# pyannote/pyannote-video

Hardware: AMD Instinct MI355X
Metric: frames/sec end-to-end detect->embed->cluster, 1080p@25fps (higher is better)
Workload: dtype f32 (detector scores, embedder) / f64 (tracker, clustering) / u8 frames; an f16 screening pass with a proven error bound decides which windows the detector's exact f32 chain is evaluated for -- results identical to dense f32 scoring (`dense_scoring`)

## Files before the change

include/pvface.h:

```cpp
#ifndef PVFACE_H
#define PVFACE_H
#include <stdint.h>
#include <stddef.h>

#ifdef __cplusplus
extern "C" {
#endif

typedef uint64_t pvf_handle;
typedef struct { int32_t left, top, right, bottom; } pvf_rect_i32;

const char* pvf_last_error(void);
int32_t pvf_version(void);
int32_t pvf_device_count(int32_t* n);
int32_t pvf_ctx_create(int32_t device, pvf_handle* ctx);
int32_t pvf_ctx_create_prio(int32_t device, int32_t priority_class, pvf_handle* ctx);
int32_t pvf_ctx_destroy(pvf_handle ctx);
int32_t pvf_sync(pvf_handle ctx);

int32_t pvf_load_detector(pvf_handle ctx, const char* path);
int32_t pvf_load_shape_predictor(pvf_handle ctx, const char* path);
int32_t pvf_load_embedder(pvf_handle ctx, const char* path);
int32_t pvf_model_tensor(const char* path, int32_t kind, const char* name, void* out, int64_t cap_bytes, int64_t* nbytes);
int32_t pvf_set_tracker_tables(pvf_handle ctx, const double* mask64, const double* mask_scale, const double* tw64,
// ... 22 lines not shown
#define PVF_PRIM_RECT 0
#define PVF_PRIM_LINE 1
#define PVF_PRIM_TEXT 2
#define PVF_RENDER_MAX_PRIMS 4096
#define PVF_RENDER_MAX_RUN 64
#define PVF_RENDER_MAX_TEXT (1 << 20)
#define PVF_RENDER_MAX_SCALE 64
#define PVF_RENDER_MAX_BATCH 1024
typedef struct { int32_t type, a, b, c, d; uint32_t colour; int32_t scale, reserved; } pvf_prim;
int32_t pvf_render_batch(pvf_handle ctx, const pvf_handle* frames, int32_t n, int32_t out_w, int32_t out_h, int32_t flags,
                         const int32_t* start, const pvf_prim* prims, const uint8_t* text, int64_t text_bytes,
                         uint8_t* out, int32_t out_on_device);
int32_t pvf_egress_create(pvf_handle ctx, int32_t out_w, int32_t out_h, int32_t depth, int32_t flags, pvf_handle* ring);
int32_t pvf_egress_destroy(pvf_handle ctx, pvf_handle ring);
int32_t pvf_egress_submit(pvf_handle ctx, pvf_handle ring, pvf_handle frame, const pvf_prim* prims, int32_t n_prims,
                          const uint8_t* text, int64_t text_bytes, int32_t* slot);
int32_t pvf_egress_wait(pvf_handle ctx, pvf_handle ring, int32_t slot, const uint8_t** host_planes);
int32_t pvf_egress_release(pvf_handle ctx, pvf_handle ring, int32_t slot);
int32_t pvf_debug_render_rgb(pvf_handle ctx, pvf_handle frame, int32_t out_w, int32_t out_h, const pvf_prim* prims, int32_t n_prims,
                             const uint8_t* text, int64_t text_bytes, uint8_t* rgb);

int32_t pvf_detect(pvf_handle ctx, pvf_handle frame, int32_t upsample, double adjust_threshold,
                   pvf_rect_i32* out, float* scores, int32_t cap, int32_t* n);
int32_t pvf_detect_batch(pvf_handle ctx, const pvf_handle* frames, int32_t n_frames, int32_t upsample,
                         double adjust_threshold, pvf_rect_i32* out, float* scores, int32_t* counts,
                         int32_t cap_per_frame);
int32_t pvf_detect_many(pvf_handle ctx, const pvf_handle* frames, int32_t n_frames, int32_t batch, int32_t upsample,
                        double adjust_threshold, pvf_rect_i32* out, float* scores, int32_t* counts, int32_t cap);

int32_t pvf_detector_screening(pvf_handle ctx, int32_t on, int32_t list_cap);
int32_t pvf_detector_screening_stats(pvf_handle ctx, int64_t* batches, int64_t* listed, int64_t* retries, double* bounds, double* pipe_err);

int32_t pvf_embedder_split(pvf_handle ctx, int32_t on);
int32_t pvf_embedder_split_stats(pvf_handle ctx, int64_t* faces, int64_t* reruns, double* pipe_err);

int32_t pvf_tracker_create(pvf_handle ctx, pvf_handle* trk);
int32_t pvf_tracker_create_many(pvf_handle ctx, int32_t n, pvf_handle* trks);
int32_t pvf_tracker_destroy_many(pvf_handle ctx, const pvf_handle* trks, int32_t n);
int32_t pvf_tracker_clone_many(pvf_handle ctx, const pvf_handle* src, int32_t n, pvf_handle* dst);
int32_t pvf_tracker_destroy(pvf_handle ctx, pvf_handle trk);
int32_t pvf_tracker_start(pvf_handle ctx, pvf_handle trk, pvf_handle frame, const double box[4]);
int32_t pvf_tracker_update(pvf_handle ctx, pvf_handle trk, pvf_handle frame, double* psr);
int32_t pvf_tracker_position(pvf_handle ctx, pvf_handle trk, double box[4]);
int32_t pvf_tracker_start_many(pvf_handle ctx, const pvf_handle* trks, const pvf_handle* frames,
                               const double* boxes , int32_t n);
int32_t pvf_tracker_update_many(pvf_handle ctx, const pvf_handle* trks, const pvf_handle* frames, int32_t n,
                                double* psr , double* boxes_out );
int32_t pvf_tracker_update_many_deferred(pvf_handle ctx, const pvf_handle* trks, const pvf_handle* frames, int32_t n,
                                         double* psr, double* boxes_out);
int32_t pvf_tracker_commit_many(pvf_handle ctx, const pvf_handle* trks, const pvf_handle* frames, int32_t n);

int32_t pvf_overlap_matrix(const double* a, int32_t na, const double* b, int32_t nb, double ratio, double* out);
int32_t pvf_associate(const double* trackers, int32_t n_trackers, const double* detections, int32_t n_detections,
                      double min_overlap_ratio, int32_t* det_of_tracker);
int32_t pvf_munkres(const double* cost, int32_t n, int32_t* row_to_col);

int32_t pvf_landmarks(pvf_handle ctx, const pvf_handle* frames, const pvf_rect_i32* boxes, int32_t n,
                      int32_t* pts );
int32_t pvf_embed(pvf_handle ctx, const pvf_handle* frames, const int32_t* pts , int32_t n,
                  float* out );
int32_t pvf_landmarks_embed(pvf_handle ctx, const pvf_handle* frames, const pvf_rect_i32* boxes, int32_t n,
                            int32_t* pts , float* out );
int32_t pvf_embed_chips(pvf_handle ctx, const uint8_t* chips, int32_t n, float* out );
int32_t pvf_face_chips(pvf_handle ctx, const pvf_handle* frames, const int32_t* pts, int32_t n, uint8_t* chips );

#define PVF_JITTER_ROW 17
// ... 113 lines not shown
```

pyannote-video_amd/csrc/api.hip:

```cpp
#include "pvf_internal.h"
#include <algorithm>
#include <cmath>
#include <cstdlib>
#include <string>
#include <thread>

#define API_BEGIN try {
#define API_END                                                        \
    return 0;                                                          \
    }                                                                  \
    catch (const std::exception& e) { pvf_set_error(e.what()); return -1; } \
    catch (...) { pvf_set_error("unknown error"); return -2; }

#define ENTER(c, h)                                                \
    Ctx* c = pvf_ctx(h);                                           \
    std::lock_guard<std::recursive_mutex> _api_lock(c->api_mu);    \
    HIP_CHECK(hipSetDevice(c->device))
#define ENTER_DET(c, h)                                            \
    Ctx* c = pvf_ctx(h);                                           \
    std::lock_guard<std::recursive_mutex> _det_lock(c->det_mu);    \
    HIP_CHECK(hipSetDevice(c->device))
#define ENTER_BOTH(c, h)                                           \
    Ctx* c = pvf_ctx(h);                                           \
    std::lock_guard<std::recursive_mutex> _det_lock(c->det_mu);    \
// ... 19 lines not shown
            with_candidate_room(c, run);
            return;
        }
    }
}

extern "C" int32_t pvf_detector_screening(pvf_handle h, int32_t on, int32_t list_cap)
{
    API_BEGIN
    ENTER_DET(c, h);
    PVF_REQUIRE(list_cap >= 0 && list_cap <= (1 << 26), "pvf_detector_screening: list_cap must be 0 (keep) .. 2^26");
    c->det_screen = on != 0;
    if (list_cap > 0) c->screen_list_cap = list_cap;
    API_END
}

extern "C" int32_t pvf_detector_screening_stats(pvf_handle h, int64_t* batches, int64_t* listed, int64_t* retries, double* bounds, double* pipe_err)
{
    API_BEGIN
    ENTER_DET(c, h);
    if (batches) *batches = c->screen_batches;
    if (listed) *listed = c->screen_listed;
    if (retries) *retries = c->screen_retries;
    if (bounds) for (int f = 0; f < c->det.n_filters; ++f) bounds[f] = c->det.screen_bound[f];
    if (pipe_err) *pipe_err = c->screen_pipe_err;
    API_END
}

extern "C" int32_t pvf_embedder_split(pvf_handle h, int32_t on)
{
    API_BEGIN
    ENTER(c, h);
    c->emb_split = on != 0;
    API_END
}

extern "C" int32_t pvf_embedder_split_stats(pvf_handle h, int64_t* faces, int64_t* reruns, double* pipe_err)
{
    API_BEGIN
    ENTER(c, h);
    if (faces) *faces = c->emb_split_faces;
    if (reruns) *reruns = c->emb_reruns;
    if (pipe_err) *pipe_err = c->emb_pipe_err;
    API_END
}

extern "C" int32_t pvf_detect_batch(pvf_handle h, const pvf_handle* frames, int32_t n_frames, int32_t upsample, double adjust,
                                    pvf_rect_i32* out, float* scores, int32_t* counts, int32_t cap)
{
    API_BEGIN
    ENTER_DET(c, h);
    PVF_REQUIRE(n_frames > 0 && frames && out && counts && cap > 0, "pvf_detect_batch: bad arguments");
    PVF_REQUIRE(upsample >= 0 && upsample <= 2, "pvf_detect_batch: upsample must be 0..2");
    std::vector<Frame> fr(n_frames);
    for (int i = 0; i < n_frames; ++i) fr[i] = c->frame(frames[i]);
    std::vector<std::vector<RawDet>> raw;
    with_candidate_room(c, [&]() { det_run_batch(c, fr, upsample, adjust, raw); });
    std::vector<RawDet> kept;
    for (int i = 0; i < n_frames; ++i) {
        det_nms(c->det, raw[i], kept);
        const int n = std::min<int>((int)kept.size(), cap);
        counts[i] = n;
        for (int k = 0; k < n; ++k) {
            out[(size_t)i * cap + k] = pvf_rect_i32{kept[k].l, kept[k].t, kept[k].rr, kept[k].b};
            if (scores) scores[(size_t)i * cap + k] = kept[k].score;
        }
// ... 1135 lines not shown
```

pyannote-video_amd/csrc/ctx.hip:

```cpp
#include "pvf_internal.h"
#include "detect_ml.h"
#include <cmath>
#include <fstream>
#include <mutex>
#include <dlfcn.h>

static thread_local std::string g_err;
void pvf_set_error(const char* msg) { g_err = msg ? msg : ""; }
extern "C" const char* pvf_last_error(void) { return g_err.c_str(); }

static std::mutex g_ctx_mu;
static std::unordered_map<uint64_t, std::unique_ptr<Ctx>> g_ctxs;
static uint64_t g_next_ctx = 0x1000;

Ctx* pvf_ctx(pvf_handle h)
{
    std::lock_guard<std::mutex> lk(g_ctx_mu);
    auto it = g_ctxs.find(h);
    if (it == g_ctxs.end()) throw PvfError("unknown context handle");
    return it->second.get();
}

std::map<std::string, Tensor> pvf_read_container(const char* path)
{
// ... 236 lines not shown
{
    API_BEGIN
    int k = 0;
    hipError_t e = hipGetDeviceCount(&k);
    if (e != hipSuccess) k = 0;
    *n = k;
    API_END
}

extern "C" int32_t pvf_ctx_create_prio(int32_t device, int32_t priority_class, pvf_handle* out)
{
    API_BEGIN
    int k = 0;
    if (hipGetDeviceCount(&k) != hipSuccess || k <= 0) throw PvfError("no HIP device visible: libpvface has no CPU fallback");
    PVF_REQUIRE(device >= 0 && device < k, "device index out of range");
    HIP_CHECK(hipSetDevice(device));
    hipDeviceProp_t prop;
    HIP_CHECK(hipGetDeviceProperties(&prop, device));
    if (strncmp(prop.gcnArchName, "gfx950", 6) != 0)
        throw PvfError(std::string("libpvface is built for gfx950 (MI355X) only; device is ") + prop.gcnArchName);
    std::unique_ptr<Ctx> c(new Ctx());
    c->device = device;
    c->n_cu = prop.multiProcessorCount;
    {
        int lo = 0, hi = 0;
        HIP_CHECK(hipDeviceGetStreamPriorityRange(&lo, &hi));
        int prio = priority_class < 0 ? lo : hi;
        if (const char* e = getenv("PVF_MAIN_STREAM_PRIO")) prio = (strcmp(e, "low") == 0) ? lo : hi;
        HIP_CHECK(hipStreamCreateWithPriority(&c->stream, hipStreamNonBlocking, priority_class == 2 ? lo : prio));
        HIP_CHECK(hipStreamCreateWithPriority(&c->det_stream, hipStreamNonBlocking, priority_class == 2 ? hi : lo));
    }
    if (const char* e = getenv("PVF_DETECTOR_SCREENING")) c->det_screen = atoi(e) != 0;
    if (const char* e = getenv("PVF_EMBEDDER_SPLIT")) c->emb_split = atoi(e) != 0;
    std::lock_guard<std::mutex> lk(g_ctx_mu);
    uint64_t id = g_next_ctx++;
    g_ctxs[id] = std::move(c);
    *out = id;
    API_END
}

extern "C" int32_t pvf_ctx_create(int32_t device, pvf_handle* out) { return pvf_ctx_create_prio(device, 0, out); }

extern "C" int32_t pvf_ctx_destroy(pvf_handle h)
{
    API_BEGIN
    Ctx* c = pvf_ctx(h);
    HIP_CHECK(hipSetDevice(c->device));
    (void)hipStreamSynchronize(c->stream);
    (void)hipStreamSynchronize(c->det_stream);
    for (auto& kv : c->frames) if (kv.second.owned) (void)hipFree((void*)kv.second.d);
    for (auto& kv : c->trackers) {
        Tracker& t = *kv.second;
        if (t.share) { if (--*t.share > 0) continue; delete t.share; t.share = nullptr; }
        if (t.d_state) (void)hipFree(t.d_state);
    }
    for (auto p : c->tracker_pool) (void)hipFree(p);
    for (int k = 0; k < 2; ++k) if (c->det_ev[k]) (void)hipEventDestroy(c->det_ev[k]);
    ml_plans_free(c);
    ingest_free_all(c);
    render_free_all(c);
    for (auto& kv : c->frame_pool) for (auto q : kv.second) {
        if (q.free_after) (void)hipEventDestroy(q.free_after);
        if (q.free_after_det) (void)hipEventDestroy(q.free_after_det);
        (void)hipFree(q.p);
    }
    if (c->d_orient_lut) (void)hipFree(c->d_orient_lut);
// ... 239 lines not shown
```

pyannote-video_amd/csrc/pvf_internal.h:

```cpp
#pragma once
#include <hip/hip_runtime.h>
#include <cstdint>
#include <cstdio>
#include <cstring>
#include <deque>
#include <map>
#include <atomic>
#include <memory>
#include <mutex>
#include <stdexcept>
#include <string>
#include <unordered_map>
#include <vector>
#include "../../include/pvface.h"
#include "scratch_layout.h"

#define PVF_FHOG_STRIDE 32

struct CandOverflow : PvfError { int needed; explicit CandOverflow(int n) : PvfError("detector: candidate buffer overflow"), needed(n) {} };
struct ScreenRetry : PvfError { ScreenRetry() : PvfError("detector: screening pass gave up") {} };

#define HIP_CHECK(expr)                                                                              \
    do {                                                                                             \
        hipError_t _e = (expr);                                                                      \
// ... 182 lines not shown
    hipStream_t stream = nullptr;
    hipStream_t det_stream = nullptr;
    DetectorModel det;
    ShapeModel shape;
    EmbedModel emb;
    TrackerTables ttab;
    std::unordered_map<uint64_t, Frame> frames;
    std::unordered_map<uint64_t, std::unique_ptr<Tracker>> trackers;
    std::vector<double*> tracker_pool;
    std::atomic<uint64_t> next_id{1};
    std::recursive_mutex api_mu;
    std::recursive_mutex det_mu;
    std::mutex frames_mu;
    std::mutex prof_mu;
    bool prof_on = false;
    std::map<std::string, ProfFamily> prof;
    std::vector<hipEvent_t> event_pool;
    DevBuf s_grad, s_pyr, s_hist, s_norm, s_feat, s_cand, s_misc, s_chip, s_chip_pyr, s_act0, s_act1, s_act2, s_trk0, s_trk1, s_trk2, s_trkfeat, s_clu0, s_clu1;
    HostBuf h_cand, h_misc;
    StageRing stage;
    DevBuf s_cand2[2], s_fptr[2];
    HostBuf h_cand2[2], h_fptr[2];
    hipEvent_t det_ev[2] = {nullptr, nullptr};
    int det_slot = 0;
    int det_cand_cap = 8192;
    bool det_screen = true, det_screen_suspended = false, screen_attr_set = false;
    int screen_list_cap = 1 << 20;
    DevBuf s_screen;
    int64_t screen_batches = 0, screen_listed = 0, screen_retries = 0;
    double screen_pipe_err = -1;
    bool screen_pipe_flushes_subnormals = false;
    bool emb_split = true, emb_probe_done = false;
    DevBuf s_emb_flags, s_emb_redo;
    DevBuf s_jit;
    bool jit_attr_set = false;
    int64_t emb_split_faces = 0, emb_reruns = 0;
    double emb_pipe_err = -1;
    int n_cu = 256;
    struct PoolBuf { uint8_t* p; hipEvent_t free_after; hipEvent_t free_after_det; };
    std::map<size_t, std::deque<PoolBuf>> frame_pool;
    size_t frame_pool_bytes = 0;
    void* ingest_rings = nullptr;
    void* render_state = nullptr;
    struct MlPlanCache* ml_plans = nullptr;
    std::map<std::vector<int>, std::unique_ptr<DevBuf>> resize_tabs;
    const void* feat_ring_owner = nullptr;
    uint8_t* d_orient_lut = nullptr;
    uint8_t* d_wrap_lut = nullptr;
    DevBuf s_orb_set, s_orb_work;
    int orb_n = 0, orb_cap = 0;

    Frame frame(uint64_t id)
    {
        std::lock_guard<std::mutex> lk(frames_mu);
        auto it = frames.find(id);
        if (it == frames.end()) throw PvfError("unknown frame handle");
        Frame& f = it->second;
        if (f.ready) {
            HIP_CHECK(hipStreamWaitEvent(stream, f.ready, 0));
            HIP_CHECK(hipStreamWaitEvent(det_stream, f.ready, 0));
            (void)hipEventDestroy(f.ready);
            f.ready = nullptr;
        }
        return f;
    }
    uint8_t* take_frame_buffer(size_t bytes, hipStream_t writer)
// ... 123 lines not shown
```

pyannote-video_amd/csrc/resnet.hip:

```cpp
#include "pvf_internal.h"
#include <cmath>
#include <cstdlib>
#include <cstring>
#include <vector>

typedef float f32x4 __attribute__((ext_vector_type(4)));
typedef uint32_t u32x4 __attribute__((ext_vector_type(4)));
typedef float f32x16 __attribute__((ext_vector_type(16)));
typedef _Float16 f16x8 __attribute__((ext_vector_type(8)));
typedef _Float16 f16x4 __attribute__((ext_vector_type(4)));
typedef uint32_t u32x2 __attribute__((ext_vector_type(2)));

void face_chip_details(const EmbedModel& m, const int32_t* pts, ChipDetails* out)
{
    const double size = m.chip_size, padding = m.chip_padding;
    double fx[51], fy[51], tx[51], ty[51];
    int n = 0;
    for (int i = 17; i < 68; ++i) {
        if ((55 <= i && i <= 59) || (65 <= i && i <= 67)) continue;
        if (17 <= i && i <= 26) continue;
        fx[n] = ((padding + (double)m.mean_shape[2 * (i - 17)]) / (2 * padding + 1)) * size;
        fy[n] = ((padding + (double)m.mean_shape[2 * (i - 17) + 1]) / (2 * padding + 1)) * size;
        tx[n] = pts[2 * i]; ty[n] = pts[2 * i + 1];
        ++n;
// ... 272 lines not shown
        __builtin_amdgcn_sched_barrier(0);
        offsets();
        Ops::chunk(pa0, pa1, pb, acc0, acc1);
        __syncthreads();
    }
    Ops::scale(a, acc0, acc1);
    conv_epilogue<WM, WN>(a, smem, acc0, acc1, M, m0, n0, rel0, b_first, hw, r_hw, r_ow, wave, lane);
}


__global__ void __launch_bounds__(256) conv_wsplit_k(const float* __restrict__ w, int total, int w_exp, _Float16* __restrict__ out)
{
    const int i = blockIdx.x * 256 + threadIdx.x;
    if (i >= total) return;
    const float v = ldexpf(w[i], w_exp);
    const _Float16 hi = (_Float16)v;
    const _Float16 lo = (_Float16)(v - (float)hi);
    const int row32 = i >> 5, kk = i & 31;
    out[(size_t)row32 * 64 + kk] = hi;
    out[(size_t)row32 * 64 + 32 + kk] = lo;
}

__global__ void __launch_bounds__(64) embed_probe_k(const uint4* __restrict__ a, const uint4* __restrict__ b, int steps, float* __restrict__ d)
{
    const int lane = threadIdx.x;
    f32x16 acc;
#pragma unroll
    for (int i = 0; i < 16; ++i) acc[i] = 0.0f;
    for (int s = 0; s < steps; ++s)
        acc = __builtin_amdgcn_mfma_f32_32x32x16_f16(__builtin_bit_cast(f16x8, a[s * 64 + lane]), __builtin_bit_cast(f16x8, b[s * 64 + lane]), acc, 0, 0, 0);
    for (int i = 0; i < 16; ++i) d[lane * 16 + i] = acc[i];
}

#define STEM_ROWS 4
#define STEM_IN_DW 1464
#define STEM_NP 77
__global__ void __launch_bounds__(64) stem_frag_k(const float* __restrict__ w, float* __restrict__ frag)
{
    const int p = blockIdx.x, l = threadIdx.x;
    const int r = p / 11, t = 2 * (p - r * 11) + (l >> 5);
    frag[p * 64 + l] = (t < 21) ? w[(size_t)(l & 31) * 224 + (r * 7 + t / 3) * 4 + t % 3] : 0.0f;
}

__global__ void __launch_bounds__(192) stem_conv_k(const uint8_t* __restrict__ chips, int B, const float* __restrict__ frag, const float* __restrict__ bias,
                                                   const float* __restrict__ gamma, const float* __restrict__ beta, float* __restrict__ out)
{
    constexpr int S = 150, OW = 72;
    __shared__ uint32_t s_in[STEM_IN_DW];
    __shared__ __attribute__((aligned(16))) float s_b[STEM_NP * 64];
    const int tid = threadIdx.x, lane = tid & 63, wave = tid >> 6;
    const int face = blockIdx.y, oy0 = blockIdx.x * STEM_ROWS;
    {
        const size_t total = (size_t)B * S * S * 3;
        const __amdgpu_buffer_rsrc_t rs = __builtin_amdgcn_make_buffer_rsrc((void*)(chips + (size_t)face * S * S * 3), 0,
                                                                             (int)std::min<size_t>(total - (size_t)face * S * S * 3, 0x7ffffff0u), 0x00020000);
        const int first = 2 * oy0 * S * 3;
        for (int i = tid; i < STEM_IN_DW; i += 192) s_in[i] = __builtin_amdgcn_raw_buffer_load_b32(rs, 4 * i, first, 0);
        const float4* f4 = reinterpret_cast<const float4*>(frag);
        float4* b4 = reinterpret_cast<float4*>(s_b);
        for (int i = tid; i < STEM_NP * 16; i += 192) b4[i] = f4[i];
    }
    __syncthreads();
    const int li = lane & 31, kh = lane >> 5;
    const uint8_t* px = reinterpret_cast<const uint8_t*>(s_in);
    const uint8_t* base[3];
#pragma unroll
    for (int t = 0; t < 3; ++t) {
        const int m = (wave * 3 + t) * 32 + li;
        const int oy = m / OW, ox = m - oy * OW;
        base[t] = px + ((2 * oy) * S + 2 * ox) * 3 + kh;
    }
    const float M0 = 122.782f, M1 = 117.001f, M2 = 104.298f;
    const float mean3[3] = {kh ? M1 : M0, kh ? M0 : M2, kh ? M2 : M1};
    f32x16 acc[3];
#pragma unroll
    for (int t = 0; t < 3; ++t)
#pragma unroll
        for (int i = 0; i < 16; ++i) acc[t][i] = 0.0f;
#pragma unroll
    for (int s = 0; s < STEM_NP; ++s) {
        const int r = s / 11, pp = s - r * 11;
        const int off = r * S * 3 + 2 * pp;
        const float b = s_b[s * 64 + lane];
#pragma unroll
        for (int t = 0; t < 3; ++t) {
            const float a = ((float)base[t][off] - mean3[pp % 3]) / 256.0f;
            acc[t] = __builtin_amdgcn_mfma_f32_32x32x2f32(a, b, acc[t], 0, 0, 0);
        }
    }
    const float bs = bias[li], g = gamma[li], bt = beta[li];
    float* o = out + ((size_t)face * OW + oy0) * OW * 32 + li;
#pragma unroll
    for (int t = 0; t < 3; ++t)
#pragma unroll
        for (int reg = 0; reg < 16; ++reg) {
            const int m = (wave * 3 + t) * 32 + (reg & 3) + 8 * (reg >> 2) + 4 * kh;
            float v = (acc[t][reg] + bs) * g + bt;
            v = v < 0.0f ? 0.0f : v;
            o[(size_t)m * 32] = v;
        }
}

#define C32_ROWS 7
#define C32_TILE_FLOATS (9 * 37 * 33)
__global__ void __launch_bounds__(64) conv_frag_k(const float* __restrict__ w, int Kpad, float* __restrict__ frag)
{
    const int s = blockIdx.x, l = threadIdx.x;
    frag[s * 64 + l] = w[(size_t)(l & 31) * Kpad + 2 * s + (l >> 5)];
}

__global__ void __launch_bounds__(256) conv3x3_c32_k(const float* __restrict__ in, const float* __restrict__ frag, const float* __restrict__ bias,
                                                     const float* __restrict__ gamma, const float* __restrict__ beta, const float* __restrict__ skip,
                                                     float* __restrict__ out, int n_items)
{
    constexpr int HW = 35, TW = 37, PITCH = 33, NP = 144;
    constexpr int NSLOT = 9 * TW * 8, PER = (NSLOT + 255) / 256;
    extern __shared__ __attribute__((aligned(16))) float smem_c32[];
    float* T = smem_c32;
    float* Bf = smem_c32 + C32_TILE_FLOATS;
    const int tid = threadIdx.x, lane = tid & 63, wave = tid >> 6;
    const int li = lane & 31, kh = lane >> 5;
    {
        const float4* f4 = reinterpret_cast<const float4*>(frag);
        float4* b4 = reinterpret_cast<float4*>(Bf);
        for (int i = tid; i < NP * 16; i += 256) b4[i] = f4[i];
    }
    const float bs = bias[li], g = gamma[li], bt = beta[li];
    const float* base[2];
#pragma unroll
    for (int t = 0; t < 2; ++t) {
        int m = (wave * 2 + t) * 32 + li;
        if (m >= C32_ROWS * HW) m = 0;
        const int oy = m / HW, ox = m - oy * HW;
// ... 279 lines not shown
    for (int k = 0; k < K; ++k)
        for (int r = 0; r < 32; ++r) {
            const float x = (float)(rnd() * 2048.0), w = (float)((rnd() * 2 - 1) * 32768.0);
            const _Float16 xh = (_Float16)x, wh = (_Float16)w;
            const float xl = x - (float)xh, wl = w - (float)wh;
            const int term = (k >> 4) % 3;
            put(r, k, r, term == 2 ? xl : (float)xh, term == 1 ? wl : (float)wh);
        }
    worst = std::max(worst, run());
    (void)hipFree(dev);
    c->emb_pipe_err = worst;
    PVF_REQUIRE(worst <= (double)K * std::ldexp(1.0, -22),
                "embed_probe: v_mfma_f32_32x32x16_f16 does not place or accumulate as the split embedder (conv_tile_k's ConvSplit) assumes on this device");
}

static const int UN[14][3] = {{32, 32, 0}, {32, 32, 0}, {32, 32, 0}, {32, 64, 1}, {64, 64, 0}, {64, 64, 0}, {64, 64, 0},
                              {64, 128, 1}, {128, 128, 0}, {128, 128, 0}, {128, 256, 1}, {256, 256, 0}, {256, 256, 0}, {256, 256, 1}};
struct UnitDims { int a, s, o; };
static UnitDims unit_dims(int u, int H)
{
    const int a = UN[u][2] ? 1 + (H - 3) / 2 : H, s = UN[u][2] ? 1 + (H - 2) / 2 : H;
    return {a, s, std::max(a, s)};
}

static void resnet_run(Ctx* c, const uint8_t* d_chips, int n, float* h_out, bool split, int* h_flags, const EmbedTap* tap = nullptr)
{
    const EmbedModel& e = c->emb;
    PVF_REQUIRE(e.loaded, "embedder not loaded");
    const int S = e.chip_size;
    const int MAXB = 4096;
    const int h1 = 1 + (S - 7) / 2;
    const int hp = 1 + (h1 - 3) / 2;
    const int cap = std::min(n, MAXB);
    const size_t big = (size_t)cap * h1 * h1 * 32;
    c->s_act0.ensure(std::max(big, (size_t)cap * S * S * 4) * sizeof(float));
    c->s_act1.ensure(big * sizeof(float));
    c->s_act2.ensure((size_t)cap * hp * hp * 32 * sizeof(float) + (size_t)cap * 128 * sizeof(float));
    PVF_REQUIRE(!tap || n <= MAXB, "embedder stage access: at most 4096 faces");
    auto tapped = [&](int stage, const float* d, int B, int H, int W, int C) {
        if (tap && tap->stage == stage && tap->h_out)
            HIP_CHECK(hipMemcpyAsync(tap->h_out, d, (size_t)B * H * W * C * sizeof(float), hipMemcpyDeviceToHost, c->stream));
    };
    for (int b0 = 0; b0 < n; b0 += MAXB) {
        const int B = std::min(MAXB, n - b0);
        ProfScope ps(c, "conv");
        float* x = c->s_act0.as<float>();
        float* y = c->s_act1.as<float>();
        float* z = c->s_act2.as<float>();
        const ConvLayer& L0 = e.convs[0];
        PVF_REQUIRE(S == 150 && L0.cout == 32 && L0.k == 7 && h1 == 72, "stem kernel: 150 x 150 chips, 7 x 7 stride 2, 32 channels");
        if (!c->emb.d_stem) {
            HIP_CHECK(hipMalloc(&c->emb.d_stem, STEM_NP * 64 * sizeof(float)));
            hipLaunchKernelGGL(stem_frag_k, dim3(STEM_NP), dim3(64), 0, c->stream, L0.d_w, c->emb.d_stem);
        }
        hipLaunchKernelGGL(stem_conv_k, dim3(h1 / STEM_ROWS, B), dim3(192), 0, c->stream, d_chips + (size_t)b0 * S * S * 3, B, c->emb.d_stem,
                           L0.d_bias, L0.d_gamma, L0.d_beta, y);
        tapped(0, y, B, h1, h1, 32);
        ConvArgs a;
        const size_t npool = (size_t)B * hp * hp * 32;
        hipLaunchKernelGGL(maxpool3s2_k, dim3((unsigned)((npool + 255) / 256)), dim3(256), 0, c->stream, y, B, h1, h1, 32, z, hp, hp);
        tapped(1, z, B, hp, hp, 32);
        float* cur = z; float* t1 = x; float* t2 = y;
        int H = hp;
        int* flags = nullptr;
        if (split) {
            flags = c->s_emb_flags.as<int>();
            HIP_CHECK(hipMemsetAsync(flags, 0, (size_t)B * sizeof(int), c->stream));
        }
        for (int u = 0; u < 14; ++u) {
            const int cin = UN[u][0], nn = UN[u][1], down = UN[u][2];
            ConvLayer& La = c->emb.convs[1 + 2 * u];
            ConvLayer& Lb = c->emb.convs[2 + 2 * u];
            const int stride = down ? 2 : 1, pad = down ? 0 : 1;
            const auto [ah, sh, oh] = unit_dims(u, H);
            memset(&a, 0, sizeof a);
            a.in = cur; a.B = B; a.H = H; a.W = H; a.Cin = cin;
            a.out = t1; a.OH = ah; a.OW = ah; a.Cout = nn; a.AH = ah; a.AW = ah; a.ksz = 3; a.stride = stride; a.pad = pad; a.skip_mode = 0;
            conv_bind_weights(c, La, split, false, flags, a);
            launch_conv(c, a);
            tapped(2 + 2 * u, t1, B, ah, ah, nn);
            memset(&a, 0, sizeof a);
            a.in = t1; a.B = B; a.H = ah; a.W = ah; a.Cin = nn;
            a.out = t2; a.OH = oh; a.OW = oh; a.Cout = nn; a.AH = ah; a.AW = ah; a.ksz = 3; a.stride = 1; a.pad = 1;
            a.skip_mode = down ? 2 : 1; a.skip = cur; a.XH = H; a.XW = H; a.XC = cin; a.SH = sh; a.SW = sh;
            conv_bind_weights(c, Lb, split, false, flags, a);
            launch_conv(c, a);
            tapped(3 + 2 * u, t2, B, oh, oh, nn);
            float* old = cur; cur = t2; t2 = old;
            H = oh;
        }
        float* d_out = reinterpret_cast<float*>(c->s_act2.as<uint8_t>() + (size_t)cap * hp * hp * 32 * sizeof(float));
        hipLaunchKernelGGL(head_k, dim3(B), dim3(256), 0, c->stream, cur, H * H, e.d_fc, d_out);
        HIP_CHECK(hipGetLastError());
// ... 126 lines not shown
```

pyannote-video_amd/pyannote_video_amd/_lib.py:

```python
import ctypes as C
import os
import numpy as np

_HERE = os.path.dirname(os.path.abspath(__file__))
LIB_PATH = os.environ.get("PVF_LIBRARY") or os.path.join(_HERE, "libpvface.so")

_lib = None


class PvfError(RuntimeError):
    pass


class OrbCapError(PvfError):

    def __init__(self, message, needed):
        PvfError.__init__(self, message)
        self.needed = int(needed)


class Rect(C.Structure):
    _fields_ = [("left", C.c_int32), ("top", C.c_int32), ("right", C.c_int32), ("bottom", C.c_int32)]


# ... 10 lines not shown
    "pvf_load_detector": (C.c_int32, [H, C.c_char_p]),
    "pvf_load_shape_predictor": (C.c_int32, [H, C.c_char_p]),
    "pvf_load_embedder": (C.c_int32, [H, C.c_char_p]),
    "pvf_model_tensor": (C.c_int32, [C.c_char_p, C.c_int32, C.c_char_p, P, C.c_int64, P]),
    "pvf_set_tracker_tables": (C.c_int32, [H, P, P, P, P, C.c_double, C.c_double]),
    "pvf_frame_upload": (C.c_int32, [H, P, C.c_int32, C.c_int32, C.c_int64, P]),
    "pvf_frame_wrap_device": (C.c_int32, [H, P, C.c_int32, C.c_int32, P]),
    "pvf_frame_release": (C.c_int32, [H, H]),
    "pvf_frame_release_many": (C.c_int32, [H, P, C.c_int32]),
    "pvf_frame_pool_trim": (C.c_int32, [H, C.c_int64, P]),
    "pvf_mem_info": (C.c_int32, [H, P, P]),
    "pvf_frame_device_ptr": (C.c_int32, [H, H, P]),
    "pvf_ingest_create": (C.c_int32, [H, C.c_int32, C.c_int32, C.c_int32, P]),
    "pvf_ingest_destroy": (C.c_int32, [H, H]),
    "pvf_ingest_acquire": (C.c_int32, [H, H, P, P]),
    "pvf_ingest_submit": (C.c_int32, [H, H, C.c_int32, P]),
    "pvf_ingest_wait": (C.c_int32, [H, H]),
    "pvf_ingest_create_yuv": (C.c_int32, [H, C.c_int32, C.c_int32, C.c_int32, C.c_int32, C.c_int32, P]),
    "pvf_frame_from_yuv": (C.c_int32, [H, P, C.c_int64, P, P, C.c_int64, C.c_int32, C.c_int32, C.c_int32, C.c_int32, C.c_int32, P]),
    "pvf_frame_resize": (C.c_int32, [H, H, C.c_int32, C.c_int32, P]),
    "pvf_render_batch": (C.c_int32, [H, P, C.c_int32, C.c_int32, C.c_int32, C.c_int32, P, P, P, C.c_int64, P, C.c_int32]),
    "pvf_egress_create": (C.c_int32, [H, C.c_int32, C.c_int32, C.c_int32, C.c_int32, P]),
    "pvf_egress_destroy": (C.c_int32, [H, H]),
    "pvf_egress_submit": (C.c_int32, [H, H, H, P, C.c_int32, P, C.c_int64, P]),
    "pvf_egress_wait": (C.c_int32, [H, H, C.c_int32, P]),
    "pvf_egress_release": (C.c_int32, [H, H, C.c_int32]),
    "pvf_debug_render_rgb": (C.c_int32, [H, H, C.c_int32, C.c_int32, P, C.c_int32, P, C.c_int64, P]),
    "pvf_detect": (C.c_int32, [H, H, C.c_int32, C.c_double, P, P, C.c_int32, P]),
    "pvf_detect_batch": (C.c_int32, [H, P, C.c_int32, C.c_int32, C.c_double, P, P, P, C.c_int32]),
    "pvf_detect_many": (C.c_int32, [H, P, C.c_int32, C.c_int32, C.c_int32, C.c_double, P, P, P, C.c_int32]),
    "pvf_detector_screening": (C.c_int32, [H, C.c_int32, C.c_int32]),
    "pvf_detector_screening_stats": (C.c_int32, [H, P, P, P, P, P]),
    "pvf_embedder_split": (C.c_int32, [H, C.c_int32]),
    "pvf_embedder_split_stats": (C.c_int32, [H, P, P, P]),
    "pvf_tracker_create": (C.c_int32, [H, P]),
    "pvf_tracker_destroy": (C.c_int32, [H, H]),
    "pvf_tracker_create_many": (C.c_int32, [H, C.c_int32, P]),
    "pvf_tracker_destroy_many": (C.c_int32, [H, P, C.c_int32]),
    "pvf_tracker_clone_many": (C.c_int32, [H, P, C.c_int32, P]),
    "pvf_tracker_start": (C.c_int32, [H, H, H, P]),
    "pvf_tracker_update": (C.c_int32, [H, H, H, P]),
    "pvf_tracker_position": (C.c_int32, [H, H, P]),
    "pvf_tracker_start_many": (C.c_int32, [H, P, P, P, C.c_int32]),
    "pvf_tracker_update_many": (C.c_int32, [H, P, P, C.c_int32, P, P]),
    "pvf_tracker_update_many_deferred": (C.c_int32, [H, P, P, C.c_int32, P, P]),
    "pvf_tracker_commit_many": (C.c_int32, [H, P, P, C.c_int32]),
    "pvf_overlap_matrix": (C.c_int32, [P, C.c_int32, P, C.c_int32, C.c_double, P]),
    "pvf_munkres": (C.c_int32, [P, C.c_int32, P]),
    "pvf_associate": (C.c_int32, [P, C.c_int32, P, C.c_int32, C.c_double, P]),
    "pvf_landmarks": (C.c_int32, [H, P, P, C.c_int32, P]),
    "pvf_embed": (C.c_int32, [H, P, P, C.c_int32, P]),
    "pvf_landmarks_embed": (C.c_int32, [H, P, P, C.c_int32, P, P]),
    "pvf_embed_chips": (C.c_int32, [H, P, C.c_int32, P]),
    "pvf_face_chips": (C.c_int32, [H, P, P, C.c_int32, P]),
    "pvf_jitter_plan": (C.c_int32, [C.c_int32, C.c_uint64, P]),
    "pvf_debug_jitter_chips": (C.c_int32, [H, P, C.c_int32, C.c_int32, C.c_uint64, P]),
    "pvf_debug_jitter_chips_transform": (C.c_int32, [H, P, C.c_int32, C.c_int32, C.c_uint64, P]),
    "pvf_embed_jitter": (C.c_int32, [H, P, P, C.c_int32, C.c_int32, C.c_uint64, P]),
    "pvf_landmarks_embed_jitter": (C.c_int32, [H, P, P, C.c_int32, C.c_int32, C.c_uint64, P, P]),
    "pvf_embed_chips_jitter": (C.c_int32, [H, P, C.c_int32, C.c_int32, C.c_uint64, P]),
    "pvf_pair_mean_dist": (C.c_int32, [H, P, C.c_int32, C.c_int32, P, C.c_int32, P]),
    "pvf_pair_mean_dist_metric": (C.c_int32, [H, P, C.c_int32, C.c_int32, P, C.c_int32, C.c_int32, P]),
    "pvf_pair_mean_dist_rows": (C.c_int32, [H, P, C.c_int32, C.c_int32, P, C.c_int32, C.c_int32, C.c_int32, P]),
    "pvf_pair_upper_rows": (C.c_int32, [H, P, C.c_int32, C.c_int32, P, C.c_int32, C.c_int32, C.c_int32, P]),
    "pvf_lane_create": (C.c_int32, [C.c_int32, P, P, C.c_int32, C.c_double, C.c_double, C.c_int32, P]),
    "pvf_lane_destroy": (C.c_int32, [H]),
# ... 191 lines not shown
```

pyannote-video_amd/pyannote_video_amd/runtime.py:

```python
import contextlib
import ctypes as C
import threading
import itertools
import operator
import numpy as np
from . import _lib
from ._lib import check, ptr, handles
from . import models as _models
from .y4m import YuvFrame, chroma_shape


class DeviceFrame(object):
    __slots__ = ("ctx", "handle", "height", "width", "keep", "transient", "__weakref__")

    def __init__(self, ctx, handle, height, width, keep=None, transient=False):
        self.ctx, self.handle, self.height, self.width, self.keep = ctx, handle, height, width, keep
        self.transient = transient

    @property
    def shape(self):
        return (self.height, self.width, 3)

    def release(self):
        if self.handle is not None and self.ctx._h is not None:
# ... 936 lines not shown
    def _cluster_dist(self, D, row_start, threshold, extent=None, flags=0):
        D = np.ascontiguousarray(D, np.float64)
        rs = np.ascontiguousarray(row_start, np.int32)
        T = len(rs) - 1
        labels = np.zeros(T, np.int32)
        log = np.zeros((max(T - 1, 1), 4), np.float64)
        n, nb = C.c_int32(0), C.c_int32(0)
        if extent is not None:
            e = self._extent(extent, T)
            check(self._l.pvf_cluster_dist_cooccur(self._h, ptr(D), ptr(rs), T, float(threshold), ptr(labels), ptr(log), C.byref(n),
                                                   ptr(e), C.byref(nb), int(flags)))
        else:
            check(self._l.pvf_cluster_dist(self._h, ptr(D), ptr(rs), T, float(threshold), ptr(labels), ptr(log), C.byref(n)))
        return labels, log[:n.value], nb.value

    def cluster_dist(self, D, row_start, threshold):
        return self._cluster_dist(D, row_start, threshold)[:2]

    def cluster_dist_cooccur(self, D, row_start, threshold, extent, flags=0):
        return self._cluster_dist(D, row_start, threshold, self._extent(extent, len(row_start) - 1), flags)

    def detector_screening(self, on=True, list_cap=0):
        check(self._l.pvf_detector_screening(self._h, 1 if on else 0, int(list_cap)))

    def detector_screening_stats(self):
        b, n, r, pe = C.c_int64(0), C.c_int64(0), C.c_int64(0), C.c_double(-1.0)
        bounds = np.zeros(8, np.float64)
        check(self._l.pvf_detector_screening_stats(self._h, C.byref(b), C.byref(n), C.byref(r), ptr(bounds), C.byref(pe)))
        return {"batches": b.value, "listed": n.value, "retries": r.value, "bounds": bounds[:5].tolist(), "pipe_err": pe.value}

    def embedder_split(self, on=True):
        check(self._l.pvf_embedder_split(self._h, 1 if on else 0))

    def embedder_split_stats(self):
        f, r, pe = C.c_int64(0), C.c_int64(0), C.c_double(-1.0)
        check(self._l.pvf_embedder_split_stats(self._h, C.byref(f), C.byref(r), C.byref(pe)))
        return {"faces": f.value, "reruns": r.value, "pipe_err": pe.value}

    def prof_enable(self, on=True):
        check(self._l.pvf_prof_enable(self._h, 1 if on else 0))

    def prof_reset(self):
        check(self._l.pvf_prof_reset(self._h))

    def prof_get(self, family):
        ms, n = C.c_double(0), C.c_int64(0)
        check(self._l.pvf_prof_get(self._h, family.encode(), C.byref(ms), C.byref(n)))
        return ms.value, n.value


def _seed64(seed):
    return int(seed) & 0xFFFFFFFFFFFFFFFF


_default = None


def default_context():
    global _default
    if _default is None:
        import os
        _default = Context(device=int(os.environ.get("LOCAL_RANK", "0")))
    return _default
```

Before: 4824.

## Fuse the 3x3 stride-2 max-pool into the embedder stem convolution kernel

Adds a pooled variant of the stem conv kernel. Each block computes 9 overlapping conv rows, parks each half of the conv output in LDS, and writes the max-pooled 35x35 map directly, replacing the separate maxpool kernel. This avoids writing and re-reading the full 72x72x32 stem activation in global memory and saves one launch. In exchange the block does redundant overlap rows and uses larger LDS with more waves. It is on by default, with a flag and env var to disable it, and falls back to the old path when stage 0 is tapped.

```diff
diff --git a/include/pvface.h b/include/pvface.h
--- a/include/pvface.h
+++ b/include/pvface.h
@@ -78,6 +78,7 @@
 int32_t pvf_detector_screening_stats(pvf_handle ctx, int64_t* batches, int64_t* listed, int64_t* retries, double* bounds, double* pipe_err);
 
 int32_t pvf_embedder_split(pvf_handle ctx, int32_t on);
+int32_t pvf_embedder_stem_pool(pvf_handle ctx, int32_t on);
 int32_t pvf_embedder_split_stats(pvf_handle ctx, int64_t* faces, int64_t* reruns, double* pipe_err);
 
 int32_t pvf_tracker_create(pvf_handle ctx, pvf_handle* trk);
diff --git a/pyannote-video_amd/csrc/api.hip b/pyannote-video_amd/csrc/api.hip
--- a/pyannote-video_amd/csrc/api.hip
+++ b/pyannote-video_amd/csrc/api.hip
@@ -75,6 +75,14 @@
     API_BEGIN
     ENTER(c, h);
     c->emb_split = on != 0;
+    API_END
+}
+
+extern "C" int32_t pvf_embedder_stem_pool(pvf_handle h, int32_t on)
+{
+    API_BEGIN
+    ENTER(c, h);
+    c->emb_stem_pool = on != 0;
     API_END
 }
 
diff --git a/pyannote-video_amd/csrc/ctx.hip b/pyannote-video_amd/csrc/ctx.hip
--- a/pyannote-video_amd/csrc/ctx.hip
+++ b/pyannote-video_amd/csrc/ctx.hip
@@ -292,6 +292,7 @@
     }
     if (const char* e = getenv("PVF_DETECTOR_SCREENING")) c->det_screen = atoi(e) != 0;
     if (const char* e = getenv("PVF_EMBEDDER_SPLIT")) c->emb_split = atoi(e) != 0;
+    if (const char* e = getenv("PVF_EMBEDDER_STEM_POOL")) c->emb_stem_pool = atoi(e) != 0;
     std::lock_guard<std::mutex> lk(g_ctx_mu);
     uint64_t id = g_next_ctx++;
     g_ctxs[id] = std::move(c);
diff --git a/pyannote-video_amd/csrc/pvf_internal.h b/pyannote-video_amd/csrc/pvf_internal.h
--- a/pyannote-video_amd/csrc/pvf_internal.h
+++ b/pyannote-video_amd/csrc/pvf_internal.h
@@ -238,6 +238,7 @@
     bool screen_pipe_flushes_subnormals = false;
     bool emb_split = true, emb_probe_done = false;
     DevBuf s_emb_flags, s_emb_redo;
+    bool emb_stem_pool = true;
     DevBuf s_jit;
     bool jit_attr_set = false;
     int64_t emb_split_faces = 0, emb_reruns = 0;
diff --git a/pyannote-video_amd/csrc/resnet.hip b/pyannote-video_amd/csrc/resnet.hip
--- a/pyannote-video_amd/csrc/resnet.hip
+++ b/pyannote-video_amd/csrc/resnet.hip
@@ -328,9 +328,26 @@
     for (int i = 0; i < 16; ++i) d[lane * 16 + i] = acc[i];
 }
 
-#define STEM_ROWS 4
-#define STEM_IN_DW 1464
 #define STEM_NP 77
+struct StemFull {
+    static constexpr bool POOL = false;
+    static constexpr int WAVES = 3, TILES = 3, ROWS = 4, STEP = 4, PW = 72, IN_DW = 1464, LDS_DW = IN_DW + STEM_NP * 64;
+};
+struct StemPool {
+    static constexpr bool POOL = true;
+    static constexpr int WAVES = 4, TILES = 5, ROWS = 9, STEP = 8, PW = 71, IN_DW = 2588;
+    static constexpr int HALF_TILES = 12, HALF_TILE0 = 8;
+    static constexpr int HALF_PX = HALF_TILES * 32, HALF_SKEW = 4 * PW - HALF_TILE0 * 32;
+    static constexpr int LDS_DW = HALF_PX * 32;
+    static constexpr int BANDS = 9, PH = 35;
+};
+static_assert(StemPool::LDS_DW >= StemPool::IN_DW + STEM_NP * 64, "stem_conv_k: the parked half overlays the chip rows and the fragments");
+static_assert(3 * StemPool::LDS_DW * 4 <= 160 * 1024, "stem_conv_k: three pooled blocks per CU (160 KB of LDS)");
+static_assert(StemPool::ROWS * StemPool::PW <= StemPool::WAVES * StemPool::TILES * 32 && StemFull::ROWS * StemFull::PW == StemFull::WAVES * StemFull::TILES * 32,
+              "stem_conv_k: the block's pixels fit its tiles");
+static_assert(StemPool::HALF_SKEW >= 0 && StemPool::HALF_SKEW + 4 * StemPool::PW + 2 * (StemPool::PH - 1) + 2 < StemPool::HALF_PX,
+              "stem_conv_k: every pixel the pool reads lies inside the parked half");
+static_assert((StemPool::IN_DW * 4) % 16 == 0 && (StemFull::IN_DW * 4) % 16 == 0, "stem_conv_k: the fragments are copied as float4");
 __global__ void __launch_bounds__(64) stem_frag_k(const float* __restrict__ w, float* __restrict__ frag)
 {
     const int p = blockIdx.x, l = threadIdx.x;
@@ -338,39 +355,42 @@
     frag[p * 64 + l] = (t < 21) ? w[(size_t)(l & 31) * 224 + (r * 7 + t / 3) * 4 + t % 3] : 0.0f;
 }
 
-__global__ void __launch_bounds__(192) stem_conv_k(const uint8_t* __restrict__ chips, int B, const float* __restrict__ frag, const float* __restrict__ bias,
-                                                   const float* __restrict__ gamma, const float* __restrict__ beta, float* __restrict__ out)
-{
-    constexpr int S = 150, OW = 72;
-    __shared__ uint32_t s_in[STEM_IN_DW];
-    __shared__ __attribute__((aligned(16))) float s_b[STEM_NP * 64];
+template <class F>
+__global__ void __launch_bounds__(F::WAVES * 64, F::POOL ? 3 : 1) stem_conv_k(const uint8_t* __restrict__ chips, int B, const float* __restrict__ frag, const float* __restrict__ bias,
+                                                             const float* __restrict__ gamma, const float* __restrict__ beta, float* __restrict__ out)
+{
+    constexpr int S = 150, NT = F::WAVES * 64, TILES = F::TILES, PW = F::PW;
+    __shared__ __attribute__((aligned(16))) uint32_t smem[F::LDS_DW];
+    uint32_t* s_in = smem;
+    float* s_b = reinterpret_cast<float*>(smem + F::IN_DW);
     const int tid = threadIdx.x, lane = tid & 63, wave = tid >> 6;
-    const int face = blockIdx.y, oy0 = blockIdx.x * STEM_ROWS;
+    const int face = blockIdx.y, oy0 = blockIdx.x * F::STEP;
     {
         const size_t total = (size_t)B * S * S * 3;
         const __amdgpu_buffer_rsrc_t rs = __builtin_amdgcn_make_buffer_rsrc((void*)(chips + (size_t)face * S * S * 3), 0,
                                                                              (int)std::min<size_t>(total - (size_t)face * S * S * 3, 0x7ffffff0u), 0x00020000);
         const int first = 2 * oy0 * S * 3;
-        for (int i = tid; i < STEM_IN_DW; i += 192) s_in[i] = __builtin_amdgcn_raw_buffer_load_b32(rs, 4 * i, first, 0);
+        for (int i = tid; i < F::IN_DW; i += NT) s_in[i] = __builtin_amdgcn_raw_buffer_load_b32(rs, 4 * i, first, 0);
         const float4* f4 = reinterpret_cast<const float4*>(frag);
         float4* b4 = reinterpret_cast<float4*>(s_b);
-        for (int i = tid; i < STEM_NP * 16; i += 192) b4[i] = f4[i];
+        for (int i = tid; i < STEM_NP * 16; i += NT) b4[i] = f4[i];
     }
     __syncthreads();
     const int li = lane & 31, kh = lane >> 5;
     const uint8_t* px = reinterpret_cast<const uint8_t*>(s_in);
-    const uint8_t* base[3];
-#pragma unroll
-    for (int t = 0; t < 3; ++t) {
-        const int m = (wave * 3 + t) * 32 + li;
-        const int oy = m / OW, ox = m - oy * OW;
+    const uint8_t* base[TILES];
+#pragma unroll
+    for (int t = 0; t < TILES; ++t) {
+        int m = (wave * TILES + t) * 32 + li;
+        if (m >= F::ROWS * PW) m = 0;
+        const int oy = m / PW, ox = m - oy * PW;
         base[t] = px + ((2 * oy) * S + 2 * ox) * 3 + kh;
     }
     const float M0 = 122.782f, M1 = 117.001f, M2 = 104.298f;
     const float mean3[3] = {kh ? M1 : M0, kh ? M0 : M2, kh ? M2 : M1};
-    f32x16 acc[3];
-#pragma unroll
-    for (int t = 0; t < 3; ++t)
+    f32x16 acc[TILES];
+#pragma unroll
+    for (int t = 0; t < TILES; ++t)
 #pragma unroll
         for (int i = 0; i < 16; ++i) acc[t][i] = 0.0f;
 #pragma unroll
@@ -379,22 +399,65 @@
         const int off = r * S * 3 + 2 * pp;
         const float b = s_b[s * 64 + lane];
 #pragma unroll
-        for (int t = 0; t < 3; ++t) {
+        for (int t = 0; t < TILES; ++t) {
             const float a = ((float)base[t][off] - mean3[pp % 3]) / 256.0f;
             acc[t] = __builtin_amdgcn_mfma_f32_32x32x2f32(a, b, acc[t], 0, 0, 0);
         }
     }
     const float bs = bias[li], g = gamma[li], bt = beta[li];
-    float* o = out + ((size_t)face * OW + oy0) * OW * 32 + li;
-#pragma unroll
-    for (int t = 0; t < 3; ++t)
-#pragma unroll
-        for (int reg = 0; reg < 16; ++reg) {
-            const int m = (wave * 3 + t) * 32 + (reg & 3) + 8 * (reg >> 2) + 4 * kh;
-            float v = (acc[t][reg] + bs) * g + bt;
-            v = v < 0.0f ? 0.0f : v;
-            o[(size_t)m * 32] = v;
-        }
+    if constexpr (!F::POOL) {
+        float* o = out + ((size_t)face * PW + oy0) * PW * 32 + li;
+#pragma unroll
+        for (int t = 0; t < TILES; ++t)
+#pragma unroll
+            for (int reg = 0; reg < 16; ++reg) {
+                const int m = (wave * TILES + t) * 32 + (reg & 3) + 8 * (reg >> 2) + 4 * kh;
+                float v = (acc[t][reg] + bs) * g + bt;
+                v = v < 0.0f ? 0.0f : v;
+                o[(size_t)m * 32] = v;
+            }
+    } else {
+        float* band = reinterpret_cast<float*>(smem);
+        constexpr int PH = F::PH;
+        const int uwave = __builtin_amdgcn_readfirstlane(wave);
+#pragma unroll 1
+        for (int half = 0; half < 2; ++half) {
+            __syncthreads();
+#pragma unroll
+            for (int t = 0; t < TILES; ++t) {
+                const int tile = uwave * TILES + t - half * F::HALF_TILE0;
+                if ((unsigned)tile < (unsigned)F::HALF_TILES) {
+                    float* d = band + (tile * 32 + 4 * kh) * 32 + li;
+#pragma unroll
+                    for (int reg = 0; reg < 16; ++reg) {
+                        float v = (acc[t][reg] + bs) * g + bt;
+                        v = v < 0.0f ? 0.0f : v;
+                        d[((reg & 3) + 8 * (reg >> 2)) * 32] = v;
+                    }
+                }
+            }
+            __syncthreads();
+            for (int o = tid; o < PH * 32; o += NT) {
+                const int ch = o & 31, q = o >> 5;
+                const float* src = band + (half * F::HALF_SKEW + 2 * q) * 32 + ch;
+                float v[5][3];
+#pragma unroll
+                for (int r = 0; r < 5; ++r)
+#pragma unroll
+                    for (int s = 0; s < 3; ++s) v[r][s] = src[(r * PW + s) * 32];
+                const int prow = blockIdx.x * 4 + 2 * half;
+#pragma unroll
+                for (int pr = 0; pr < 2; ++pr) {
+                    float mx = -INFINITY;
+#pragma unroll
+                    for (int r = 0; r < 3; ++r)
+#pragma unroll
+                        for (int s = 0; s < 3; ++s) mx = fmaxf(mx, v[2 * pr + r][s]);
+                    if (prow + pr < PH) out[(((size_t)face * PH + prow + pr) * PH + q) * 32 + ch] = mx;
+                }
+            }
+        }
+    }
 }
 
 #define C32_ROWS 7
@@ -740,10 +803,11 @@
     const int h1 = 1 + (S - 7) / 2;
     const int hp = 1 + (h1 - 3) / 2;
     const int cap = std::min(n, MAXB);
-    const size_t big = (size_t)cap * h1 * h1 * 32;
-    c->s_act0.ensure(std::max(big, (size_t)cap * S * S * 4) * sizeof(float));
-    c->s_act1.ensure(big * sizeof(float));
-    c->s_act2.ensure((size_t)cap * hp * hp * 32 * sizeof(float) + (size_t)cap * 128 * sizeof(float));
+    const bool pooled = c->emb_stem_pool && !(tap && tap->stage == 0);
+    const size_t unit = (size_t)cap * hp * hp * 32;
+    c->s_act0.ensure(unit * sizeof(float));
+    c->s_act1.ensure((pooled ? unit : (size_t)cap * h1 * h1 * 32) * sizeof(float));
+    c->s_act2.ensure(unit * sizeof(float) + (size_t)cap * 128 * sizeof(float));
     PVF_REQUIRE(!tap || n <= MAXB, "embedder stage access: at most 4096 faces");
     auto tapped = [&](int stage, const float* d, int B, int H, int W, int C) {
         if (tap && tap->stage == stage && tap->h_out)
@@ -756,17 +820,22 @@
         float* y = c->s_act1.as<float>();
         float* z = c->s_act2.as<float>();
         const ConvLayer& L0 = e.convs[0];
-        PVF_REQUIRE(S == 150 && L0.cout == 32 && L0.k == 7 && h1 == 72, "stem kernel: 150 x 150 chips, 7 x 7 stride 2, 32 channels");
+        PVF_REQUIRE(S == 150 && L0.cout == 32 && L0.k == 7 && h1 == 72 && hp == StemPool::PH, "stem kernel: 150 x 150 chips, 7 x 7 stride 2, 32 channels");
         if (!c->emb.d_stem) {
             HIP_CHECK(hipMalloc(&c->emb.d_stem, STEM_NP * 64 * sizeof(float)));
             hipLaunchKernelGGL(stem_frag_k, dim3(STEM_NP), dim3(64), 0, c->stream, L0.d_w, c->emb.d_stem);
         }
-        hipLaunchKernelGGL(stem_conv_k, dim3(h1 / STEM_ROWS, B), dim3(192), 0, c->stream, d_chips + (size_t)b0 * S * S * 3, B, c->emb.d_stem,
-                           L0.d_bias, L0.d_gamma, L0.d_beta, y);
-        tapped(0, y, B, h1, h1, 32);
         ConvArgs a;
-        const size_t npool = (size_t)B * hp * hp * 32;
-        hipLaunchKernelGGL(maxpool3s2_k, dim3((unsigned)((npool + 255) / 256)), dim3(256), 0, c->stream, y, B, h1, h1, 32, z, hp, hp);
+        if (pooled) {
+            hipLaunchKernelGGL(stem_conv_k<StemPool>, dim3(StemPool::BANDS, B), dim3(StemPool::WAVES * 64), 0, c->stream, d_chips + (size_t)b0 * S * S * 3, B,
+                               c->emb.d_stem, L0.d_bias, L0.d_gamma, L0.d_beta, z);
+        } else {
+            hipLaunchKernelGGL(stem_conv_k<StemFull>, dim3(h1 / StemFull::ROWS, B), dim3(StemFull::WAVES * 64), 0, c->stream, d_chips + (size_t)b0 * S * S * 3, B,
+                               c->emb.d_stem, L0.d_bias, L0.d_gamma, L0.d_beta, y);
+            tapped(0, y, B, h1, h1, 32);
+            const size_t npool = (size_t)B * hp * hp * 32;
+            hipLaunchKernelGGL(maxpool3s2_k, dim3((unsigned)((npool + 255) / 256)), dim3(256), 0, c->stream, y, B, h1, h1, 32, z, hp, hp);
+        }
         tapped(1, z, B, hp, hp, 32);
         float* cur = z; float* t1 = x; float* t2 = y;
         int H = hp;
diff --git a/pyannote-video_amd/pyannote_video_amd/_lib.py b/pyannote-video_amd/pyannote_video_amd/_lib.py
--- a/pyannote-video_amd/pyannote_video_amd/_lib.py
+++ b/pyannote-video_amd/pyannote_video_amd/_lib.py
@@ -66,6 +66,7 @@
     "pvf_detector_screening": (C.c_int32, [H, C.c_int32, C.c_int32]),
     "pvf_detector_screening_stats": (C.c_int32, [H, P, P, P, P, P]),
     "pvf_embedder_split": (C.c_int32, [H, C.c_int32]),
+    "pvf_embedder_stem_pool": (C.c_int32, [H, C.c_int32]),
     "pvf_embedder_split_stats": (C.c_int32, [H, P, P, P]),
     "pvf_tracker_create": (C.c_int32, [H, P]),
     "pvf_tracker_destroy": (C.c_int32, [H, H]),
diff --git a/pyannote-video_amd/pyannote_video_amd/runtime.py b/pyannote-video_amd/pyannote_video_amd/runtime.py
--- a/pyannote-video_amd/pyannote_video_amd/runtime.py
+++ b/pyannote-video_amd/pyannote_video_amd/runtime.py
@@ -992,6 +992,9 @@
     def embedder_split(self, on=True):
         check(self._l.pvf_embedder_split(self._h, 1 if on else 0))
 
+    def embedder_stem_pool(self, on=True):
+        check(self._l.pvf_embedder_stem_pool(self._h, 1 if on else 0))
+
     def embedder_split_stats(self):
         f, r, pe = C.c_int64(0), C.c_int64(0), C.c_double(-1.0)
         check(self._l.pvf_embedder_split_stats(self._h, C.byref(f), C.byref(r), C.byref(pe)))
```

Result: slower. 4734 (-1.9%).
